# OmerShubi/DL_VQA

Measured on AMD Instinct MI355X. Metric: VQA samples/sec (train step), higher is better.
Workload: dtype f32; 1 GPU; VqaNet train step (fwd+softCE+bwd+Adam), batch 256/GPU, 224x224 images, 14-token questions, 1000-way head, train mode; global_batch=256, image_size=224, answers=1000, vocab=5000, parallelism=dp1

## Files before the change

### dl_vqa_amd/csrc/conv_patch_f32.hip

```cpp
#include "bf16_core.hpp"
#include <stdlib.h>

namespace vqa {

constexpr int PF_WMAX = 256;

template <int WM_>
struct PfCfg {
  static constexpr int WM = WM_, WN = 8 / WM_;
  static constexpr int SEG = 128 * WM;
  static constexpr int NSLAB = 64 * WN;
  static constexpr int PLANE = SEG + 2 * (PF_WMAX + 2) + 8;
  static constexpr int PATCH_BYTES = ((8 * PLANE * 4 + 1023) / 1024) * 1024;
  static constexpr int W_BYTES = 9 * 8 * NSLAB * 4;
  static constexpr int W_INSTR = W_BYTES / 1024;
  static constexpr int WK = (W_INSTR + 7) / 8;
  static constexpr int LDS = 2 * (PATCH_BYTES + W_BYTES);
  static constexpr int RT_K = 2;
};

struct PfParams {
  const char* dp;
  const char* am;
  const char* wimg;
  float* out;
  int B, Cin, N, H, W, Wp2, Hq, Wq;
  int EW;
  int segs, nunits;
  int nslabs, nslices;
  int dbg;
};

typedef unsigned int pf_rsrc_t __attribute__((ext_vector_type(4)));
__device__ __forceinline__ pf_rsrc_t pf_rsrc(const void* base, uint32_t bytes = 0xffff0000u) {
  const uint64_t a = (uint64_t)base;
  pf_rsrc_t r;
  r.x = __builtin_amdgcn_readfirstlane((uint32_t)a);
  r.y = __builtin_amdgcn_readfirstlane((uint32_t)(a >> 32) & 0xffffu);
  r.z = __builtin_amdgcn_readfirstlane(bytes);
  r.w = 0x00020000u;
  return r;
}
__device__ __forceinline__ void pf_dma16(pf_rsrc_t r, const void* lds_dst, uint32_t voff, uint32_t soff) {
  const uint32_t m0v = __builtin_amdgcn_readfirstlane((uint32_t)(uintptr_t)(__attribute__((address_space(3))) const char*)lds_dst);
  uint32_t keep;
  asm volatile("s_nop 4\n\ts_mov_b32 %0, m0\n\ts_mov_b32 m0, %1\n\ts_nop 0\n\tbuffer_load_dwordx4 %2, %3, %4 offen lds\n\ts_mov_b32 m0, %0"
               : "=&s"(keep) : "s"(m0v), "v"(voff), "s"(r), "s"(soff) : "memory");
}

template <int WMv>
__global__ __launch_bounds__(512, 2) void pconvf_dgrad_kernel(const PfParams P) {
  using C = PfCfg<WMv>;
  extern __shared__ __attribute__((aligned(1024))) char smem[];
  const int lane = threadIdx.x & 63;
  const int wave = __builtin_amdgcn_readfirstlane(threadIdx.x >> 6);
  const int wm = wave / C::WN, wn = wave % C::WN;
  const int r = lane & 31, h = lane >> 5;

  const int bid = blockIdx.x;
  const int slab = (bid >> 3) % P.nslabs;
  const int stream = ((bid >> 3) / P.nslabs) * 8 + (bid & 7);
  const int nstreams = gridDim.x / P.nslabs;
  const int my_tiles = stream < P.nunits ? (P.nunits - stream + nstreams - 1) / nstreams : 0;
  if (my_tiles == 0) return;
  const int n_slab0 = slab * C::NSLAB;
  const int PLEN = C::SEG + 2 * P.Wp2 + 2;

  const uint32_t a_lane = (uint32_t)((h * C::PLANE + wm * 128 + r) * 4);
  const uint32_t b_lane = (uint32_t)(2 * C::PATCH_BYTES + (h * C::NSLAB + wn * 64 + r) * 4);

  const pf_rsrc_t wrs = pf_rsrc(P.wimg);
  const uint32_t wlane = (uint32_t)lane * 16u;
  uint32_t ns_wsrc = 0;
  int ns_buf = 0;
  bool ns_on = false;
  auto issue_piece = [&](int n) {
    if (!ns_on) return;
    const int i = wave + 8 * n;
    if (n < C::WK && i < C::W_INSTR)
      pf_dma16(wrs, smem + 2 * C::PATCH_BYTES + ns_buf * C::W_BYTES + i * 1024, wlane, ns_wsrc + i * 1024);
  };

  int t_er[C::RT_K], t_e[C::RT_K];
#pragma unroll
  for (int k = 0; k < C::RT_K; ++k) {
    const int t = k * 512 + (int)threadIdx.x;
    t_er[k] = t / P.EW;
    t_e[k] = t - t_er[k] * P.EW;
  }
  float4 rt_d0[C::RT_K], rt_d1[C::RT_K];
  uint2 rt_a[C::RT_K];
  int rt_unit = stream, rt_slice = 0, rt_count = 0;
  const int rt_total = my_tiles * P.nslices;
  auto rt_load = [&]() {
    const bool on = rt_count < rt_total;
    const int img = rt_unit / P.segs, seg = rt_unit - img * P.segs;
    const int er0 = (seg * C::SEG / P.Wp2) >> 1;
    const int64_t ibase = (int64_t)img * P.Hq * P.Wq * P.Cin;
    const uint32_t ibytes = (uint32_t)(P.Hq * P.Wq * P.Cin);
    const __amdgpu_buffer_rsrc_t rd = buf_rsrc(P.dp + ibase * 4, ibytes * 4u), ra = buf_rsrc(P.am + ibase, ibytes);
#pragma unroll
    for (int k = 0; k < C::RT_K; ++k) {
      const int qy = er0 + t_er[k] - 1, qx = t_e[k] - 1;
      const bool ok = on && (unsigned)qy < (unsigned)P.Hq && (unsigned)qx < (unsigned)P.Wq;
      const uint32_t o = (uint32_t)((qy * P.Wq + qx) * P.Cin + 8 * rt_slice);
      rt_d0[k] = buf_load16(rd, ok ? o * 4u : BUF_OOB);
      rt_d1[k] = buf_load16(rd, ok ? o * 4u + 16u : BUF_OOB);
      rt_a[k] = buf_load8(ra, ok ? o : BUF_OOB);
    }
    ++rt_count;
    if (++rt_slice == P.nslices) { rt_slice = 0; rt_unit += nstreams; }
  };
  auto rt_route = [&](int buf, int p0) {
    char* const dst = smem + buf * C::PATCH_BYTES;
    const int er0 = (p0 / P.Wp2) >> 1;
#pragma unroll
    for (int k = 0; k < C::RT_K; ++k) {
      const float d[8] = {rt_d0[k].x, rt_d0[k].y, rt_d0[k].z, rt_d0[k].w, rt_d1[k].x, rt_d1[k].y, rt_d1[k].z, rt_d1[k].w};
      const int yy = 2 * (er0 + t_er[k]), xx = 2 * t_e[k];
#pragma unroll
      for (int j = 0; j < 4; ++j) {
        const int pl = (yy + (j >> 1)) * P.Wp2 + xx + (j & 1) - p0;
        if (xx + (j & 1) < P.Wp2 && pl >= 0 && pl < PLEN) {
#pragma unroll
          for (int ch = 0; ch < 8; ++ch) {
            const uint32_t code = ((ch < 4 ? rt_a[k].x : rt_a[k].y) >> (8 * (ch & 3))) & 0xffu;
            *reinterpret_cast<float*>(dst + (ch * C::PLANE + pl) * 4) = code == (uint32_t)j ? d[ch] : 0.f;
          }
        }
      }
    }
  };

  f32x16 acc[4][2];
  auto zero_acc = [&]() {
#pragma unroll
    for (int i = 0; i < 4; ++i)
#pragma unroll
      for (int j = 0; j < 2; ++j)
#pragma unroll
        for (int e = 0; e < 16; ++e) acc[i][j][e] = 0.f;
  };
  zero_acc();

  uint32_t toff[9];
#pragma unroll
  for (int t = 0; t < 9; ++t) toff[t] = (uint32_t)(((t / 3) * P.Wp2 + t % 3) * 4);

  ns_wsrc = (uint32_t)((slab * P.nslices + 0) * C::W_BYTES);
  ns_buf = 0;
  ns_on = true;
#pragma unroll
  for (int n = 0; n < C::WK; ++n) issue_piece(n);
  rt_load();
  rt_route(0, (stream % P.segs) * C::SEG);
  rt_load();
  int buf = 0, gstage = 0;
  int unit = stream;
  for (int k = 0; k < my_tiles; ++k, unit += nstreams) {
    const int img = unit / P.segs, seg = unit - img * P.segs;
    const int p0 = seg * C::SEG;
    for (int slice = 0; slice < P.nslices; ++slice, ++gstage) {
      asm volatile("s_waitcnt vmcnt(0) lgkmcnt(0)" ::: "memory");
      __builtin_amdgcn_s_barrier();
      const bool last_slice = slice + 1 == P.nslices;
      {
        ns_wsrc = (uint32_t)((slab * P.nslices + (last_slice ? 0 : slice + 1)) * C::W_BYTES);
        ns_buf = buf ^ 1;
        ns_on = gstage + 1 < rt_total;
      }
      const int np0 = last_slice ? ((unit + nstreams) % P.segs) * C::SEG : p0;
      const char* const pa = smem + buf * C::PATCH_BYTES + a_lane;
      const char* const pb = smem + buf * C::W_BYTES + b_lane;
      float a[2][4], b[2][2];
      auto fetch = [&](int t, int ks, int set) {
        const char* const pat = pa + toff[t];
#pragma unroll
        for (int i = 0; i < 4; ++i) a[set][i] = *reinterpret_cast<const float*>(pat + ((2 * ks) * C::PLANE + 32 * i) * 4);
#pragma unroll
        for (int j = 0; j < 2; ++j)
          b[set][j] = *reinterpret_cast<const float*>(pb + ((t * 8 + 2 * ks) * C::NSLAB + 32 * j) * 4);
      };
      fetch(0, 0, 0);
#pragma unroll
      for (int t = 0; t < 9; ++t) {
#pragma unroll
        for (int ks = 0; ks < 4; ++ks) {
          const int q = 4 * t + ks;
          if (q + 1 < 36) fetch((q + 1) >> 2, (q + 1) & 3, (q + 1) & 1);
          __builtin_amdgcn_sched_barrier(0);
#pragma unroll
          for (int i = 0; i < 4; ++i)
#pragma unroll
            for (int j = 0; j < 2; ++j)
              acc[i][j] = __builtin_amdgcn_mfma_f32_32x32x2f32(a[q & 1][i], b[q & 1][j], acc[i][j], 0, 0, 0);
          __builtin_amdgcn_sched_barrier(0);
        }
        __builtin_amdgcn_sched_barrier(0);
        if (t == 0) { if (ns_on && !(P.dbg & 1)) rt_route(buf ^ 1, np0); }
        else if (t == 1) rt_load();
        else if (t < 2 + C::WK) { if (!(P.dbg & 2)) issue_piece(t - 2); }
        __builtin_amdgcn_sched_barrier(0);
      }
      buf ^= 1;
    }
    const int64_t obase = (int64_t)img * P.H * P.W * P.N + n_slab0 + wn * 64;
    const __amdgpu_buffer_rsrc_t ro = buf_rsrc(P.out + obase);
#pragma unroll
    for (int i = 0; i < 4; ++i)
#pragma unroll
      for (int e = 0; e < 16; ++e) {
        const int m = p0 + wm * 128 + 32 * i + (e & 3) + 8 * (e >> 2) + 4 * h;
        const int y = m / P.Wp2, x = m - y * P.Wp2;
        const bool ok = x < P.W && y < P.H && !(P.dbg & 4);
        const uint32_t vo = ok ? (uint32_t)(((y * P.W + x) * P.N + r) * 4) : BUF_OOB;
#pragma unroll
        for (int j = 0; j < 2; ++j) buf_store4(ro, acc[i][j][e], vo, (uint32_t)(32 * j * 4));
      }
    zero_acc();
  }
}

__global__ void pconvf_pack_kernel(const float* w, float* img, int Co, int Ci, int nslab) {
  const int64_t total = (int64_t)9 * Ci * Co;
  const int64_t idx = (int64_t)blockIdx.x * blockDim.x + threadIdx.x;
  if (idx >= total) return;
  const int n = (int)(idx % nslab);
  int64_t t = idx / nslab;
  const int k = (int)(t % 8); t /= 8;
  const int tap = (int)(t % 9); t /= 9;
  const int nslices = Co / 8;
  const int slice = (int)(t % nslices);
  const int slab = (int)(t / nslices);
  const int ky = tap / 3, kx = tap - 3 * ky;
  const int co = 8 * slice + k, ci = slab * nslab + n;
  img[idx] = w[((int64_t)co * Ci + ci) * 9 + (2 - ky) * 3 + (2 - kx)];
}

static int pf_nslab(int N) { return N % 128 == 0 ? 128 : 64; }

template <int WMv>
static int pf_launch(PfParams P, hipStream_t s) {
  using C = PfCfg<WMv>;
  P.segs = (P.H * P.Wp2 + C::SEG - 1) / C::SEG;
  P.nunits = P.B * P.segs;
  auto kern = pconvf_dgrad_kernel<WMv>;
  int rc = ensure_dyn_smem(reinterpret_cast<const void*>(kern), C::LDS, "attr(pconvf_dgrad)");
  if (rc) return rc;
  int grid = 256;
  grid -= grid % (8 * P.nslabs);
  hipLaunchKernelGGL(kern, dim3(grid), dim3(512), C::LDS, s, P);
  return check_hip(hipGetLastError(), "pconvf_dgrad launch");
}

}

using namespace vqa;

extern "C" {

int vqa_pconvf_supported(int H, int W, int Ci, int Co, int stride) {
  if (stride != 1 || H < 4 || W < 4 || W > PF_WMAX || Ci % 64 || Co % 8 || Ci <= 0 || Co <= 0 || Ci > 4096 || Co > 4096) return 0;
  if (256 % (8 * (Ci / pf_nslab(Ci)))) return 0;
  if ((int64_t)H * W * (Ci > Co ? Ci : Co) * 4 >= (1LL << 31)) return 0;
  const int Wp2 = W + 2, seg = pf_nslab(Ci) == 128 ? 512 : 1024;
  const int rows = (seg + 2 * Wp2 + 2) / Wp2 + 2;
  if ((rows / 2 + 2) * ((Wp2 + 1) / 2) > 1024) return 0;
  return 1;
}

int64_t vqa_pconvf_weights_bytes(int Ci, int Co) { return (int64_t)9 * Ci * Co * 4; }

int vqa_pconvf_pack_weights(const float* w, float* wd_img, int Co, int Ci, vqa_stream_t stream) {
  VQA_REQUIRE(w && wd_img && Ci % 64 == 0 && Co % 8 == 0, "vqa_pconvf_pack_weights: bad args Co=%d Ci=%d", Co, Ci);
  const int64_t total = (int64_t)9 * Ci * Co;
  hipLaunchKernelGGL(pconvf_pack_kernel, dim3((unsigned)((total + 255) / 256)), dim3(256), 0, (hipStream_t)stream, w, wd_img, Co, Ci,
                     pf_nslab(Ci));
  return check_hip(hipGetLastError(), "pconvf_pack launch");
}

int vqa_pconvf_dgrad(const float* dpooled, const uint8_t* argmax, const float* wd_img, float* dx, int B, int H, int W, int Ci, int Co,
                     int tag, vqa_stream_t stream) {
  VQA_REQUIRE(dpooled && argmax && wd_img && dx && B > 0, "vqa_pconvf_dgrad: null pointer");
  VQA_REQUIRE(vqa_pconvf_supported(H, W, Ci, Co, 1), "vqa_pconvf_dgrad: unsupported shape H=%d W=%d Ci=%d Co=%d", H, W, Ci, Co);
  PfParams P{};
  P.dp = reinterpret_cast<const char*>(dpooled);
  P.am = reinterpret_cast<const char*>(argmax);
  P.wimg = reinterpret_cast<const char*>(wd_img);
  P.out = dx;
  P.B = B; P.Cin = Co; P.N = Ci; P.H = H; P.W = W; P.Wp2 = W + 2;
  P.Hq = (H - 2) / 2; P.Wq = (W - 2) / 2;
  VQA_REQUIRE(P.Hq > 0 && P.Wq > 0, "vqa_pconvf_dgrad: image too small");
  P.EW = (P.Wp2 + 1) / 2;
  const int nslab = pf_nslab(Ci);
  P.nslabs = Ci / nslab;
  P.nslices = Co / 8;
  {
    const char* e = getenv("VQA_PCONVF_DBG");
    P.dbg = e ? atoi(e) : 0;
  }
  hipStream_t s = (hipStream_t)stream;
  set_launch_tag(tag);
  ProfScope prof(VQA_K_CONV_DGRAD, s);
  return nslab == 128 ? pf_launch<4>(P, s) : pf_launch<8>(P, s);
}

}
```

Before: 9762 samples/s.

## Interleave wave M rows and skip MFMA for partial tail tiles in conv dgrad

The fused pool/conv data-gradient kernel now interleaves wave row ownership (wm*32 stride with 32*WM step), so a partially filled last segment maps to fewer active i-blocks. A per-tile compile-time variant (NI=1..4) then skips MFMAs and stores for the empty rows at the tail. The grid size is now taken from an occupancy-based persistent slot count instead of a fixed 256, and the debug env lookup and flags are compiled out unless VQA_DIAG is defined. Instantiating four variants grows code size and instruction-cache footprint, and the new grid size changes how work is split across CUs.

```diff
diff --git a/dl_vqa_amd/csrc/conv_patch_f32.hip b/dl_vqa_amd/csrc/conv_patch_f32.hip
--- a/dl_vqa_amd/csrc/conv_patch_f32.hip
+++ b/dl_vqa_amd/csrc/conv_patch_f32.hip
@@ -28,8 +28,15 @@
   int EW;
   int segs, nunits;
   int nslabs, nslices;
+#ifdef VQA_DIAG
   int dbg;
+#endif
 };
+#ifdef VQA_DIAG
+#define PF_DBG(bit) ((P.dbg & (bit)) != 0)
+#else
+#define PF_DBG(bit) false
+#endif
 
 typedef unsigned int pf_rsrc_t __attribute__((ext_vector_type(4)));
 __device__ __forceinline__ pf_rsrc_t pf_rsrc(const void* base, uint32_t bytes = 0xffff0000u) {
@@ -66,7 +73,7 @@
   const int n_slab0 = slab * C::NSLAB;
   const int PLEN = C::SEG + 2 * P.Wp2 + 2;
 
-  const uint32_t a_lane = (uint32_t)((h * C::PLANE + wm * 128 + r) * 4);
+  const uint32_t a_lane = (uint32_t)((h * C::PLANE + wm * 32 + r) * 4);
   const uint32_t b_lane = (uint32_t)(2 * C::PATCH_BYTES + (h * C::NSLAB + wn * 64 + r) * 4);
 
   const pf_rsrc_t wrs = pf_rsrc(P.wimg);
@@ -156,8 +163,8 @@
   rt_route(0, (stream % P.segs) * C::SEG);
   rt_load();
   int buf = 0, gstage = 0;
-  int unit = stream;
-  for (int k = 0; k < my_tiles; ++k, unit += nstreams) {
+  auto run_tile = [&](auto ni_const, int unit) __attribute__((always_inline)) {
+    constexpr int NI = decltype(ni_const)::value;
     const int img = unit / P.segs, seg = unit - img * P.segs;
     const int p0 = seg * C::SEG;
     for (int slice = 0; slice < P.nslices; ++slice, ++gstage) {
@@ -172,11 +179,12 @@
       const int np0 = last_slice ? ((unit + nstreams) % P.segs) * C::SEG : p0;
       const char* const pa = smem + buf * C::PATCH_BYTES + a_lane;
       const char* const pb = smem + buf * C::W_BYTES + b_lane;
-      float a[2][4], b[2][2];
+      float a[2][NI], b[2][2];
       auto fetch = [&](int t, int ks, int set) {
         const char* const pat = pa + toff[t];
 #pragma unroll
-        for (int i = 0; i < 4; ++i) a[set][i] = *reinterpret_cast<const float*>(pat + ((2 * ks) * C::PLANE + 32 * i) * 4);
+        for (int i = 0; i < NI; ++i)
+          a[set][i] = *reinterpret_cast<const float*>(pat + ((2 * ks) * C::PLANE + 32 * C::WM * i) * 4);
 #pragma unroll
         for (int j = 0; j < 2; ++j)
           b[set][j] = *reinterpret_cast<const float*>(pb + ((t * 8 + 2 * ks) * C::NSLAB + 32 * j) * 4);
@@ -190,34 +198,51 @@
           if (q + 1 < 36) fetch((q + 1) >> 2, (q + 1) & 3, (q + 1) & 1);
           __builtin_amdgcn_sched_barrier(0);
 #pragma unroll
-          for (int i = 0; i < 4; ++i)
+          for (int i = 0; i < NI; ++i)
 #pragma unroll
             for (int j = 0; j < 2; ++j)
               acc[i][j] = __builtin_amdgcn_mfma_f32_32x32x2f32(a[q & 1][i], b[q & 1][j], acc[i][j], 0, 0, 0);
           __builtin_amdgcn_sched_barrier(0);
         }
         __builtin_amdgcn_sched_barrier(0);
-        if (t == 0) { if (ns_on && !(P.dbg & 1)) rt_route(buf ^ 1, np0); }
+        if (t == 0) { if (ns_on && !PF_DBG(1)) rt_route(buf ^ 1, np0); }
         else if (t == 1) rt_load();
-        else if (t < 2 + C::WK) { if (!(P.dbg & 2)) issue_piece(t - 2); }
+        else if (t < 2 + C::WK) { if (!PF_DBG(2)) issue_piece(t - 2); }
         __builtin_amdgcn_sched_barrier(0);
       }
       buf ^= 1;
     }
     const int64_t obase = (int64_t)img * P.H * P.W * P.N + n_slab0 + wn * 64;
     const __amdgpu_buffer_rsrc_t ro = buf_rsrc(P.out + obase);
-#pragma unroll
-    for (int i = 0; i < 4; ++i)
+    int m0 = p0 + 32 * wm + 4 * h;
+    asm volatile("" : "+v"(m0));
+#pragma unroll
+    for (int i = 0; i < NI; ++i)
 #pragma unroll
       for (int e = 0; e < 16; ++e) {
-        const int m = p0 + wm * 128 + 32 * i + (e & 3) + 8 * (e >> 2) + 4 * h;
+        const int m = m0 + 32 * C::WM * i + (e & 3) + 8 * (e >> 2);
         const int y = m / P.Wp2, x = m - y * P.Wp2;
-        const bool ok = x < P.W && y < P.H && !(P.dbg & 4);
+        const bool ok = x < P.W && y < P.H && !PF_DBG(4);
         const uint32_t vo = ok ? (uint32_t)(((y * P.W + x) * P.N + r) * 4) : BUF_OOB;
 #pragma unroll
         for (int j = 0; j < 2; ++j) buf_store4(ro, acc[i][j][e], vo, (uint32_t)(32 * j * 4));
       }
-    zero_acc();
+#pragma unroll
+    for (int i = 0; i < NI; ++i)
+#pragma unroll
+      for (int j = 0; j < 2; ++j)
+#pragma unroll
+        for (int e = 0; e < 16; ++e) acc[i][j][e] = 0.f;
+  };
+  const int npos = P.H * P.Wp2;
+  int unit = stream;
+  for (int k = 0; k < my_tiles; ++k, unit += nstreams) {
+    const int left = npos - (unit % P.segs) * C::SEG;
+    const int ni = __builtin_amdgcn_readfirstlane(left >= C::SEG ? 4 : (left + 32 * C::WM - 1) / (32 * C::WM));
+    if (ni == 4) run_tile(std::integral_constant<int, 4>{}, unit);
+    else if (ni == 3) run_tile(std::integral_constant<int, 3>{}, unit);
+    else if (ni == 2) run_tile(std::integral_constant<int, 2>{}, unit);
+    else run_tile(std::integral_constant<int, 1>{}, unit);
   }
 }
 
@@ -247,8 +272,10 @@
   auto kern = pconvf_dgrad_kernel<WMv>;
   int rc = ensure_dyn_smem(reinterpret_cast<const void*>(kern), C::LDS, "attr(pconvf_dgrad)");
   if (rc) return rc;
-  int grid = 256;
+  int grid = persistent_slots(reinterpret_cast<const void*>(kern), 512, C::LDS, 1);
+  if (grid <= 0) return VQA_ERR_HIP;
   grid -= grid % (8 * P.nslabs);
+  VQA_REQUIRE(grid > 0, "pconvf_dgrad: %d channel slabs need at least %d compute units", P.nslabs, 8 * P.nslabs);
   hipLaunchKernelGGL(kern, dim3(grid), dim3(512), C::LDS, s, P);
   return check_hip(hipGetLastError(), "pconvf_dgrad launch");
 }
@@ -295,10 +322,10 @@
   const int nslab = pf_nslab(Ci);
   P.nslabs = Ci / nslab;
   P.nslices = Co / 8;
-  {
-    const char* e = getenv("VQA_PCONVF_DBG");
-    P.dbg = e ? atoi(e) : 0;
-  }
+#ifdef VQA_DIAG
+  static const int dbg = [] { const char* e = getenv("VQA_PCONVF_DBG"); return e ? atoi(e) : 0; }();
+  P.dbg = dbg;
+#endif
   hipStream_t s = (hipStream_t)stream;
   set_launch_tag(tag);
   ProfScope prof(VQA_K_CONV_DGRAD, s);
```

Result: no change. 9850 samples/s (median of 6 runs) (+0.9%).
